# Atten4Vis/LW-DETR

Hardware: AMD Instinct MI355X
Metric: images/sec (higher is better)
Workload: dtype fp16; 1 GPU; LW-DETR-small inference forward + PostProcess, 640x640, batch 32/GPU, fp16, random-init weights (synthetic COCO-shaped input); global_batch=32, per_gpu_batch=32, parallelism=dp1, collective=none, launch_chains=2

## Files before the change

include/lwdetr_hip.h:

```cpp
#ifndef LWDETR_HIP_H
#define LWDETR_HIP_H
#include <stdint.h>
#ifdef __cplusplus
extern "C" {
#endif

#define LWDETR_OK 0
#define LWDETR_ERR_BAD_ARG (-1)
#define LWDETR_ERR_UNSUPPORTED (-2)
#define LWDETR_ERR_LAUNCH (-3)

int lwdetr_msda_forward(const void* value, const int64_t* shapes, const int64_t* level_start, const void* loc,
                        const void* attn, void* out, int B, int S, int M, int D, int L, int Q, int P, int dtype,
                        void* hip_stream);

int lwdetr_msda_backward(const void* value, const int64_t* shapes, const int64_t* level_start, const void* loc,
                         const void* attn, const void* grad_out, void* grad_value, void* grad_loc, void* grad_attn,
                         int B, int S, int M, int D, int L, int Q, int P, int dtype, void* hip_stream);

int lwdetr_msda_fused_forward(const void* value, const int64_t* shapes, const int64_t* level_start, const void* oa,
                              long ld_oa, int logit_col, const float* ref_boxes, const float* valid_ratios, void* out,
                              int B, int S, int M, int D, int L, int Q, int P, int dtype, void* hip_stream);

typedef struct {
// ... 41 lines not shown
    lwdetr_gemm_seg seg[3];
    void* splitk_ws;
    int splitk;
} lwdetr_gemm_desc;

int lwdetr_gemm(const lwdetr_gemm_desc* desc, int dtype, void* hip_stream);
int lwdetr_gemm_few(const lwdetr_gemm_desc* desc, int dtype, void* hip_stream);
int lwdetr_row_stats(const void* x, long ldx, long M, int C, float eps, float* stats, int dtype, void* hip_stream);
void lwdetr_gemm_tuning(int big_mode);
int lwdetr_has_experiments(void);
void lwdetr_gemm_pt_tuning(int pt_mode);
long lwdetr_gemm_pt_count(void);
int lwdetr_gemm_path_counts(long* out, int n);
const char* lwdetr_gemm_path_name(int i);

typedef struct {
    const void* Q;
    const void* K;
    const void* VT;
    void* out;
    long ldo;
    int B, heads, hd, Tp;
    int seqs_per_img;
    int seq_tok_stride;
    int keys_per_seq;
    int sub_stride, sub_len;
    int kind;
    int vt_slack;
} lwdetr_attn_desc;

int lwdetr_attention(const lwdetr_attn_desc* desc, int dtype, void* hip_stream);
void lwdetr_attention_tuning(int lds_mode);
void lwdetr_attention_tuning_cfg(int cfg);

int lwdetr_layernorm(const void* x, long ldx, const float* gamma, const float* beta, void* out, long ldo, long M,
                     int C, float eps, long rows_per_batch, long out_batch_rows, long out_row_offset, int dtype,
                     void* hip_stream);

int lwdetr_layernorm_chain(const void* x, long ldx, const float* gamma1, const float* beta1, float eps1, void* out1, long ldo1,
                           const float* gamma2, const float* beta2, float eps2, void* out2, long ldo2, long M, int C,
                           int dtype, void* hip_stream);

int lwdetr_ffn_splits(long M, int C, int hid, int dtype);
int lwdetr_ffn_partial(const void* x, long ldx, const void* w1, const float* b1, const void* w2_chunked, float* partial, long M,
                       int C, int hid, int dtype, void* hip_stream);
int lwdetr_ffn_finish(const void* x, long ldx, const float* partial, int splits, const float* b2, const float* gamma1,
                      const float* beta1, float eps1, void* out1, long ldo1, const float* gamma2, const float* beta2, float eps2,
                      void* out2, long ldo2, long M, int C, int dtype, void* hip_stream);

int lwdetr_mlp_fused(void* x, long ldx, const void* w1_folded, const float* b1_folded, const void* w2_chunked,
                     const float* b2, const float* gamma2, void* out2, long ld2, float* stats_out, long M, int C,
                     float eps, float eps_next, const void* att, long ldatt, const void* wp, const float* bp,
                     const float* gamma1, const void* wqkv_next, const float* bqkv_next, void* q_out, void* k_out,
                     void* vt_out, float qscale, int heads, int hd, int Tp, int dtype, void* hip_stream);

int lwdetr_vit_block_few(void* x, long ldx, const void* w1_frag, const float* b1_folded, const void* w2_chunked, const float* b2,
                         const float* gamma2, void* out2, long ld2, float* stats_out, long M, int C, float eps, float eps_next,
                         const void* att, long ldatt, const void* wp_frag, const float* bp, const float* gamma1,
                         const void* wqkv_frag_next, const float* bqkv_next, void* q_out, void* k_out, void* vt_out, float qscale,
                         int heads, int hd, int Tp, int dtype, void* hip_stream);

long lwdetr_vit_block_stream_bytes(int C, int has_qkv);
long lwdetr_vit_block_vec_floats(int C);
int lwdetr_vit_block(void* x, long ldx, const void* att, long ldatt, const void* wstream, const float* vec, void* out2,
                     long ld2, float* stats_out, long M, int C, float eps, float eps_next, int has_qkv, void* q_out,
                     void* k_out, void* vt_out, float qscale, int heads, int hd, int Tp, int dtype, void* hip_stream);
// ... 74 lines not shown
```

lw-detr_amd/csrc/attention.hip:

```cpp
#include "common.h"
#include <cstdlib>

namespace {

__device__ __forceinline__ float xor16_max(float v) {
    const auto r = __builtin_amdgcn_permlane16_swap(__float_as_uint(v), __float_as_uint(v), false, false);
    return fmaxf(__uint_as_float(r[0]), __uint_as_float(r[1]));
}
__device__ __forceinline__ float xor32_max(float v) {
    const auto r = __builtin_amdgcn_permlane32_swap(__float_as_uint(v), __float_as_uint(v), false, false);
    return fmaxf(__uint_as_float(r[0]), __uint_as_float(r[1]));
}
__device__ __forceinline__ float xor16_sum(float v) {
    const auto r = __builtin_amdgcn_permlane16_swap(__float_as_uint(v), __float_as_uint(v), false, false);
    return __uint_as_float(r[0]) + __uint_as_float(r[1]);
}
__device__ __forceinline__ float xor32_sum(float v) {
    const auto r = __builtin_amdgcn_permlane32_swap(__float_as_uint(v), __float_as_uint(v), false, false);
    return __uint_as_float(r[0]) + __uint_as_float(r[1]);
}

__device__ __forceinline__ float max3(float a, float b, float c) { return __builtin_fmaxf(__builtin_fmaxf(a, b), c); }

#ifndef LWDETR_ATTN_ABL
#define LWDETR_ATTN_ABL 0
#endif

template <typename T, int HD, int QT, bool SHORT = false>
__global__ __launch_bounds__(256) void attn_kernel(const lwdetr_attn_desc p) {
    typedef typename Vec<T>::v8 V8;
    typedef typename Vec<T>::v4 V4;
    constexpr int NC = HD >= 32 ? HD / 32 : 1;
    constexpr int DT = HD / 16;
    const int lane = threadIdx.x & 63, wave = threadIdx.x >> 6;
// ... 202 lines not shown
    }
}


template <typename T> struct Mma32;
template <> struct Mma32<f16> {
    static __device__ __forceinline__ f32x16 k16(f16x8 a, f16x8 b, f32x16 c) {
        return __builtin_amdgcn_mfma_f32_32x32x16_f16(a, b, c, 0, 0, 0);
    }
    static __device__ __forceinline__ float dot2(f16x8 p, int i, float c) {
        typedef _Float16 h2 __attribute__((ext_vector_type(2)));
        const h2 a = {p[2 * i], p[2 * i + 1]}, one = {(f16)1.f, (f16)1.f};
        return __builtin_amdgcn_fdot2(a, one, c, false);
    }
};
template <> struct Mma32<bf16> {
    static __device__ __forceinline__ f32x16 k16(bf16x8 a, bf16x8 b, f32x16 c) {
        return __builtin_amdgcn_mfma_f32_32x32x16_bf16(a, b, c, 0, 0, 0);
    }
    static __device__ __forceinline__ float dot2(bf16x8 p, int i, float c) {
        typedef __bf16 b2 __attribute__((ext_vector_type(2)));
        const b2 a = {p[2 * i], p[2 * i + 1]}, one = {(bf16)1.f, (bf16)1.f};
        return __builtin_amdgcn_fdot2_f32_bf16(a, one, c, false);
    }
};

__device__ __attribute__((aligned(16))) unsigned int g_attn_zero16[4];

__device__ __forceinline__ void attn_dma16(const void* src, unsigned lds_base) {
    asm volatile("s_mov_b32 m0, %0\n\ts_nop 0\n\tglobal_load_lds_dwordx4 %1, off" :: "s"(lds_base), "v"(src) : "memory");
}
template <int N> __device__ __forceinline__ void attn_wait_vmcnt() { asm volatile("s_waitcnt vmcnt(%0)" ::"n"(N) : "memory"); }

template <typename T, int HD, int QT, int NW, int U>
__global__ __launch_bounds__(NW * 64) void attn_lds_kernel(const lwdetr_attn_desc p) {
    typedef typename Vec<T>::v8 V8;
    constexpr int NC = HD / 16;
    constexpr int RT = HD > 32 ? HD / 32 : 1;
    constexpr int RB = HD * 2;
    constexpr int CPR = RB / 16, RPB = 256 / RB;
    constexpr int KB = 64;
    constexpr int KIMG = KB * RB, VIMG = RT * 32 * 128, STAGE = KIMG + VIMG;
    constexpr int NKP = KIMG / 1024, NVP = HD * 128 / 1024, NP = NKP + NVP;
    constexpr int SSTAGE = U * STAGE;
    constexpr int PPW = (U * NP + NW - 1) / NW;
    constexpr int NST = 3;
    constexpr int QW = 32 * QT, QWG = QW * NW;
    constexpr float RESCALE_THR = 8.f;
    __shared__ __attribute__((aligned(16))) char smem[NST * SSTAGE + 1024];

    const int lane = threadIdx.x & 63;
    const int wave = __builtin_amdgcn_readfirstlane(threadIdx.x >> 6);
    const int m = lane & 31, h = lane >> 5;
    const int nkeys = p.keys_per_seq;
    const int wgs_per_seq = (nkeys + QWG - 1) / QWG;
    int wid;
    {
        const int nwg = gridDim.x, bid = blockIdx.x, q = nwg >> 3, r = nwg & 7, xcd = bid & 7;
        wid = (xcd < r ? xcd * (q + 1) : r * (q + 1) + (xcd - r) * q) + (bid >> 3);
    }
    const int qblk = wid % wgs_per_seq;
    const int rest = wid / wgs_per_seq;
    const int head = rest % p.heads, seq = rest / p.heads;
    const int b = seq / p.seqs_per_img, w = seq - b * p.seqs_per_img;
    const long tok0 = (long)w * p.seq_tok_stride;
    const long bh = (long)b * p.heads + head;
    const T* __restrict__ Qb = (const T*)p.Q + (bh * p.Tp + tok0) * HD;
// ... 62 lines not shown
    const int km = (m & ~12) | ((m & 4) << 1) | ((m & 8) >> 1);
    int kofs[NC];
#pragma unroll
    for (int c = 0; c < NC; ++c) kofs[c] = km * RB + (((2 * c + h) ^ ((km / RPB) & (CPR - 1))) << 4);
    int vofs[2][2];
#pragma unroll
    for (int t = 0; t < 2; ++t)
#pragma unroll
        for (int s = 0; s < 2; ++s) vofs[t][s] = KIMG + m * 128 + (((4 * t + 2 * s + h) ^ ((m >> 1) & 7)) << 4);

    f32x16 o[QT][RT], negm[QT];
    float lsum[QT];
#pragma unroll
    for (int t = 0; t < QT; ++t) {
        lsum[t] = 0.f;
#pragma unroll
        for (int e = 0; e < 16; ++e) negm[t][e] = 0.f;
#pragma unroll
        for (int r = 0; r < RT; ++r)
#pragma unroll
            for (int e = 0; e < 16; ++e) o[t][r][e] = 0.f;
    }
    const bool holes = p.sub_len < p.sub_stride;
    int res0 = 0;

#pragma unroll
    for (int s = 0; s < NST - 1; ++s) issue(s, s);
#pragma unroll
    for (int t = 0; t < QT; ++t)
#pragma unroll
        for (int c = 0; c < NC; ++c) asm volatile("" :: "v"(qf[t][c]));

    int slot = 0;
    for (int ks = 0; ks < nstep; ++ks) {
        asm volatile("s_waitcnt lgkmcnt(0)" ::: "memory");
        attn_wait_vmcnt<(NST - 2) * PPW>();
        __builtin_amdgcn_s_barrier();
        {
            int ns = slot + NST - 1; ns = ns >= NST ? ns - NST : ns;
            issue(ks + NST - 1, ns);
        }
        const char* sS = smem + slot * SSTAGE;
        slot = slot + 1 == NST ? 0 : slot + 1;
#pragma unroll
        for (int u = 0; u < U; ++u) {
        const int kb = ks * U + u;
        if (kb >= nblk) break;
        const char* sK = sS + u * STAGE;
        if (active) {
#pragma unroll
            for (int t = 0; t < 2; ++t) {
                V8 kf[NC], vf[2][RT];
#pragma unroll
                for (int c = 0; c < NC; ++c) kf[c] = *(const V8*)(sK + t * 32 * RB + kofs[c]);
#pragma unroll
                for (int s = 0; s < 2; ++s)
#pragma unroll
                    for (int r = 0; r < RT; ++r) vf[s][r] = *(const V8*)(sK + r * 4096 + vofs[t][s]);
                f32x16 sc[QT];
#pragma unroll
                for (int qt = 0; qt < QT; ++qt) {
                    f32x16 a = negm[qt];
#pragma unroll
                    for (int c = 0; c < NC; ++c) a = Mma32<T>::k16(kf[c], qf[qt][c], a);
                    sc[qt] = a;
                }
// ... 28 lines not shown
                        float mx = xor32_max(lmax[qt]);
                        mx = first ? mx : fmaxf(mx, 0.f);
                        const float alpha = __builtin_amdgcn_exp2f(-mx);
#pragma unroll
                        for (int e = 0; e < 16; ++e) { negm[qt][e] -= mx; sc[qt][e] -= mx; }
                        lsum[qt] *= alpha;
#pragma unroll
                        for (int r = 0; r < RT; ++r)
#pragma unroll
                            for (int e = 0; e < 16; ++e) o[qt][r][e] *= alpha;
                    }
                }
#pragma unroll
                for (int qt = 0; qt < QT; ++qt) {
                    V8 pf[2];
#pragma unroll
                    for (int e = 0; e < 16; ++e) pf[e >> 3][e & 7] = from_f32<T>(__builtin_amdgcn_exp2f(sc[qt][e]));
                    if (HD > 16) {
#pragma unroll
                        for (int s = 0; s < 2; ++s)
#pragma unroll
                            for (int i = 0; i < 4; ++i) lsum[qt] = Mma32<T>::dot2(pf[s], i, lsum[qt]);
                    }
#pragma unroll
                    for (int s = 0; s < 2; ++s)
#pragma unroll
                        for (int r = 0; r < RT; ++r) o[qt][r] = Mma32<T>::k16(vf[s][r], pf[s], o[qt][r]);
                }
            }
        } else {
            res0 += 64; res0 %= p.sub_stride;
        }
        }
    }
    attn_wait_vmcnt<0>();
    if (!active) return;

    T* __restrict__ out = (T*)p.out;
#pragma unroll
    for (int qt = 0; qt < QT; ++qt) {
        float l;
        if (HD == 16) {
            const unsigned x = __float_as_uint(o[qt][0][8]);
            const auto rr = __builtin_amdgcn_permlane32_swap(x, x, false, false);
            l = __uint_as_float(rr[0]);
        } else {
            l = xor32_sum(lsum[qt]);
        }
        const float inv = 1.f / l;
        const int q = q0 + qt * 32 + m;
        T* orow = out + ((long)b * p.Tp + tok0 + q) * p.ldo + head * HD;
#pragma unroll
        for (int r = 0; r < RT; ++r)
#pragma unroll
            for (int j = 0; j < (HD == 16 ? 1 : 2); ++j) {
                typedef typename Vec<T>::v4 V4;
                V4 a4, b4;
#pragma unroll
                for (int e = 0; e < 4; ++e) {
                    a4[e] = from_f32<T>(o[qt][r][8 * j + e] * inv);
                    b4[e] = from_f32<T>(o[qt][r][8 * j + 4 + e] * inv);
                }
                typedef unsigned u2 __attribute__((ext_vector_type(2)));
                u2 au = __builtin_bit_cast(u2, a4), bu = __builtin_bit_cast(u2, b4);
#pragma unroll
                for (int d = 0; d < 2; ++d) {
                    const auto sw = __builtin_amdgcn_permlane32_swap(au[d], bu[d], false, false);
                    au[d] = sw[0]; bu[d] = sw[1];
                }
                typedef unsigned u4 __attribute__((ext_vector_type(4)));
                const u4 st = {au[0], au[1], bu[0], bu[1]};
                if (q < nkeys) *(u4*)(orow + r * 32 + j * 16 + h * 8) = st;
            }
    }
}

template <typename T, int HD, int QT, int NW, int U = 1>
int launch_lds(const lwdetr_attn_desc& p, hipStream_t st) {
    if constexpr (3 * U * (64 * HD * 2 + (HD > 32 ? HD / 32 : 1) * 32 * 128) + 1024 > 65536) return LWDETR_ERR_UNSUPPORTED;
    else {
    const int wgs_per_seq = (p.keys_per_seq + 32 * QT * NW - 1) / (32 * QT * NW);
    const long nwg = (long)wgs_per_seq * p.heads * p.B * p.seqs_per_img;
    const double nseq = (double)p.B * p.seqs_per_img;
    const double flops = 4.0 * nseq * p.heads * (double)p.keys_per_seq * p.keys_per_seq * HD;
    const double bytes = 4.0 * nseq * p.heads * p.keys_per_seq * HD * sizeof(T);
    ProfScope ps(p.kind == 0 ? KID_ATTN_WINDOW : (p.kind == 1 ? KID_ATTN_GLOBAL : KID_ATTN_DECODER), flops, bytes, st);
    hipLaunchKernelGGL((attn_lds_kernel<T, HD, QT, NW, U>), dim3((unsigned)nwg), dim3(NW * 64), 0, st, p);
    return lwdetr_check_launch();
    }
}

int g_attn_lds_cfg = 0;
}
extern "C" __attribute__((visibility("hidden"))) int lwdetr_attn_lds_hd16_impl(const lwdetr_attn_desc* p, int dtype, void* hip_stream, int cfg);
namespace {
template <typename T, int HD>
int launch_lds_cfg(const lwdetr_attn_desc& p, hipStream_t st) {
    int c = g_attn_lds_cfg ? g_attn_lds_cfg : (int)lwdetr_knob(KNOB_ATTN_LDS_CFG, 0);
#ifndef LWDETR_ATTN_HD16_TU
    if constexpr (HD == 16) return lwdetr_attn_lds_hd16_impl(&p, std::is_same<T, f16>::value ? DT_F16 : DT_BF16, (void*)st, c);
    else {
#else
    {
#endif
    if (!c) c = p.keys_per_seq <= 128 || HD == 16 ? 104 : (HD >= 64 && p.keys_per_seq >= 512 ? 208 : 108);
    switch (c) {
        case 102: return launch_lds<T, HD, 1, 2>(p, st);
        case 103: return launch_lds<T, HD, 1, 3>(p, st);
        case 104: return launch_lds<T, HD, 1, 4>(p, st);
        case 105: return launch_lds<T, HD, 1, 5>(p, st);
        case 106: return launch_lds<T, HD, 1, 6>(p, st);
        case 108: return launch_lds<T, HD, 1, 8>(p, st);
        case 110: return launch_lds<T, HD, 1, 10>(p, st);
        case 204: return launch_lds<T, HD, 2, 4>(p, st);
        case 205: return launch_lds<T, HD, 2, 5>(p, st);
        case 208: return launch_lds<T, HD, 2, 8>(p, st);
        case 1104: return launch_lds<T, HD, 1, 4, 2>(p, st);
        case 1105: return launch_lds<T, HD, 1, 5, 2>(p, st);
        case 1108: return launch_lds<T, HD, 1, 8, 2>(p, st);
        case 1110: return launch_lds<T, HD, 1, 10, 2>(p, st);
        case 3108: return launch_lds<T, HD, 1, 8, 4>(p, st);
        case 1208: return launch_lds<T, HD, 2, 8, 2>(p, st);
        default: return LWDETR_ERR_UNSUPPORTED;
    }
    }
}
template <typename T, int HD> struct LdsPath {
    static bool ok(const lwdetr_attn_desc&) { return false; }
    static int go(const lwdetr_attn_desc&, hipStream_t) { return LWDETR_ERR_UNSUPPORTED; }
};
template <int HD> struct LdsPath<f16, HD> {
    static bool ok(const lwdetr_attn_desc& p) { return true; }
    static int go(const lwdetr_attn_desc& p, hipStream_t st) { return launch_lds_cfg<f16, HD>(p, st); }
};
template <int HD> struct LdsPath<bf16, HD> {
    static bool ok(const lwdetr_attn_desc& p) { return true; }
    static int go(const lwdetr_attn_desc& p, hipStream_t st) { return launch_lds_cfg<bf16, HD>(p, st); }
};
// ... 365 lines not shown
    if constexpr (sizeof(T) == 2 && (HD == 16 || HD == 32)) {
        const int mode = (int)lwdetr_knob(KNOB_ATTN_WIN, 2);
        if (mode != 0 && (mode == 1 || HD == 32) && p.keys_per_seq <= 128 && p.sub_stride >= p.keys_per_seq && p.ldo % 8 == 0 &&
            ((size_t)p.out & 15) == 0 && (long)p.B * p.heads * p.seqs_per_img / 4 < 0x7fffffffL)
            return launch_win<T, HD>(p, st);
    }
    if (LdsPath<T, HD>::ok(p) && lds_path_applies(p)) return LdsPath<T, HD>::go(p, st);
    const long wgs4 = (long)((p.keys_per_seq + 255) / 256) * p.heads * p.B * p.seqs_per_img;
    const bool qt4 = lwdetr_knob_is_set(KNOB_ATTN_QT) ? lwdetr_knob(KNOB_ATTN_QT, 0) == 4 : (p.keys_per_seq >= 1024 && HD <= 32 && sizeof(T) == 2 && wgs4 >= 256);
    if (qt4) return launch_qt<T, HD, (HD <= 32 ? 4 : 2)>(p, st);
    return launch_qt<T, HD, 2>(p, st);
}

template <typename T>
int dispatch_hd(const lwdetr_attn_desc& p, hipStream_t st) {
    switch (p.hd) {
        case 16: return launch<T, 16>(p, st);
        case 32: return launch<T, 32>(p, st);
        case 64: return launch<T, 64>(p, st);
        default: return LWDETR_ERR_UNSUPPORTED;
    }
}

}

#ifdef LWDETR_ATTN_HD16_TU
extern "C" __attribute__((visibility("hidden"))) int lwdetr_attn_lds_hd16_impl(const lwdetr_attn_desc* p, int dtype, void* hip_stream, int cfg) {
    g_attn_lds_cfg = cfg;
    return dtype == DT_F16 ? launch_lds_cfg<f16, 16>(*p, (hipStream_t)hip_stream) : launch_lds_cfg<bf16, 16>(*p, (hipStream_t)hip_stream);
}
#else
extern "C" void lwdetr_attention_tuning(int lds_mode) { g_attn_lds_mode = lds_mode; }
extern "C" void lwdetr_attention_tuning_cfg(int cfg) { g_attn_lds_cfg = cfg; }

extern "C" int lwdetr_attention(const lwdetr_attn_desc* desc, int dtype, void* hip_stream) {
    if (!desc) return LWDETR_ERR_BAD_ARG;
    const lwdetr_attn_desc& p = *desc;
    if (!p.Q || !p.K || !p.VT || !p.out || p.B <= 0 || p.heads <= 0 || p.Tp <= 0 || p.Tp % 4 != 0) return LWDETR_ERR_BAD_ARG;
    if (p.seqs_per_img <= 0 || p.keys_per_seq < 8 || p.keys_per_seq % 4 != 0 || p.sub_stride <= 0 || p.sub_len <= 0 || p.sub_len > p.sub_stride)
        return LWDETR_ERR_BAD_ARG;
    if ((long)(p.seqs_per_img - 1) * p.seq_tok_stride + p.keys_per_seq > p.Tp) return LWDETR_ERR_BAD_ARG;
    if (p.seq_tok_stride % 4 != 0 || p.ldo % 4 != 0) return LWDETR_ERR_BAD_ARG;
    if ((long)p.B * p.seqs_per_img > 65535 || p.heads > 65535) return LWDETR_ERR_BAD_ARG;
    hipStream_t st = (hipStream_t)hip_stream;
    switch (dtype) {
        case DT_F32: return dispatch_hd<float>(p, st);
        case DT_F16: return dispatch_hd<f16>(p, st);
        case DT_BF16: return dispatch_hd<bf16>(p, st);
        default: return LWDETR_ERR_UNSUPPORTED;
    }
}
#endif
```

lw-detr_amd/csrc/vitblock.hip:

```cpp
#include "common.h"
#include <cstdlib>
#include <cstring>
#include <type_traits>

#ifndef LWDETR_VB_ABLATE
#define LWDETR_VB_ABLATE 0
#endif
#ifdef LWDETR_VB_TIMING
__device__ unsigned long long g_vb_timing[2][4][16];
#define VB_TS(i) do { if ((blockIdx.x == 0 || blockIdx.x == gridDim.x - 1) && lane == 0) { g_vb_timing[blockIdx.x != 0][wave][i] = __builtin_amdgcn_s_memrealtime(); \
    if ((i) == 0) g_vb_timing[blockIdx.x != 0][wave][12] = __builtin_amdgcn_s_memtime(); if ((i) == 11) g_vb_timing[blockIdx.x != 0][wave][15] = __builtin_amdgcn_s_memtime(); } } while (0)
extern "C" int lwdetr_debug_vb_timing(unsigned long long* out) {
    return hipMemcpyFromSymbol(out, HIP_SYMBOL(g_vb_timing), sizeof(g_vb_timing)) == hipSuccess ? 0 : 1;
}
#else
#define VB_TS(i) do {} while (0)
#endif

namespace {

template <typename T> struct Mma32;
template <> struct Mma32<f16> {
    static __device__ __forceinline__ f32x16 k16(f16x8 a, f16x8 b, f32x16 c) { return __builtin_amdgcn_mfma_f32_32x32x16_f16(a, b, c, 0, 0, 0); }
};
// ... 149 lines not shown
        if (ioff == NSLOT * PIECE_B) ioff = 0;
    };
    auto issued_is = [&](int n) { issued = n; isrc = wsrc + (size_t)n * PIECE_B; ioff = (unsigned)(n % NSLOT) * PIECE_B; };
#ifdef LWDETR_VB_TIMING
    unsigned long long tt_wait = 0, tt_bar = 0;
#endif
    auto boundary = [&](int a, int b, int extra) {
        __builtin_amdgcn_sched_barrier(0);
#ifdef LWDETR_VB_TIMING
        const unsigned long long ta = __builtin_amdgcn_s_memrealtime();
#endif
        vb_wait_le<(NSLOT - 4) * DPW>((issued - b) * DPW + extra);
#ifdef LWDETR_VB_TIMING
        const unsigned long long tb = __builtin_amdgcn_s_memrealtime();
#endif
        asm volatile("s_waitcnt lgkmcnt(0)" ::: "memory");
        __builtin_amdgcn_s_barrier();
#ifdef LWDETR_VB_TIMING
        tt_wait += tb - ta; tt_bar += __builtin_amdgcn_s_memrealtime() - tb;
#endif
        int lim = a + NSLOT; lim = lim < NP ? lim : NP;
#if LWDETR_VB_ABLATE & 4
        if (a >= H0) { issued = lim; return; }
#endif
        while (issued < lim) dma_next();
    };
    auto frag = [&](int piece, int f) -> V8 {
        return *(const V8*)(smem + ((unsigned)piece % NSLOT) * PIECE_B + f * 1024 + lane16);
    };
    auto frag_o = [&](unsigned off, int f) -> V8 { return *(const V8*)(smem + off + f * 1024 + lane16); };
    auto next_off = [](unsigned off) { off += PIECE_B; return off == NSLOT * PIECE_B ? 0u : off; };

    VB_TS(0);
    {
        const char* vsrc = (const char*)p.vec;
#pragma unroll
        for (int i = 0; i < VEC_DPW; ++i) {
            const unsigned kb = (unsigned)(wave * VEC_DPW + i) * 1024u;
            dma1k(vsrc, kb + lane16, lds0 + NSLOT * PIECE_B + kb);
        }
        while (issued < NSLOT) dma_next();
    }
    const T* att_w = (const T*)p.att + t0 * p.ldatt;
    T* x_w = (T*)p.x + t0 * p.ldx;
    const __amdgpu_buffer_rsrc_t r_att = __builtin_amdgcn_make_buffer_rsrc((void*)att_w, 0, (int)(nvalid * p.ldatt * 2), 0x00020000);
    const __amdgpu_buffer_rsrc_t r_x = __builtin_amdgcn_make_buffer_rsrc((void*)x_w, 0, (int)(nvalid * p.ldx * 2), 0x00020000);
    V8 xf[NH][KS];
#pragma unroll
    for (int th = 0; th < NH; ++th)
#pragma unroll
        for (int t = 0; t < KS; ++t)
            xf[th][t] = __builtin_bit_cast(V8, __builtin_amdgcn_raw_buffer_load_b128(
                r_att, (unsigned)(((32 * th + j) * p.ldatt + 16 * t + 8 * h) * 2), 0, 0));

    f32x16 acc2[NTI][NH];
    {
        u32x4 xv[NH][NTI][2];
#pragma unroll
        for (int th = 0; th < NH; ++th)
#pragma unroll
            for (int n = 0; n < NTI; ++n)
#pragma unroll
                for (int jb = 0; jb < 2; ++jb)
                    xv[th][n][jb] = __builtin_amdgcn_raw_buffer_load_b128(
                        r_x, (unsigned)(((32 * th + j) * p.ldx + 32 * n + 16 * jb + 8 * h) * 2), 0, 0);
        boundary(0, 2, NH * KS + NH * NTI * 2);
        VB_TS(1);
#pragma unroll
        for (int n = 0; n < NTI; ++n) {
            f32x16 na[NH];
#pragma unroll
            for (int jb = 0; jb < 2; ++jb)
#pragma unroll
                for (int th = 0; th < NH; ++th) {
                    const u32x4 own = vb_rows8(xv[th][n][jb][0], xv[th][n][jb][1], xv[th][n][jb][2], xv[th][n][jb][3]);
#pragma unroll
                    for (int bb = 0; bb < 2; ++bb) {
                        const int b = 2 * jb + bb, c0 = 32 * n + 8 * b + 4 * h;
                        const f32x4 bbv = *(const f32x4*)(bps + c0), rg = *(const f32x4*)(rg1s + c0);
#pragma unroll
                        for (int d = 0; d < 2; ++d) {
                            const unsigned ow_ = own[2 * bb + d];
                            const typename Pk<T>::v2 v2 = __builtin_bit_cast(typename Pk<T>::v2, ow_);
                            na[th][4 * b + 2 * d] = fmaf(to_f32<T>(v2[0]), rg[2 * d], bbv[2 * d]);
                            na[th][4 * b + 2 * d + 1] = fmaf(to_f32<T>(v2[1]), rg[2 * d + 1], bbv[2 * d + 1]);
                        }
                    }
                }
#pragma unroll
            for (int th = 0; th < NH; ++th) {
                asm volatile("" : "+a"(na[th]));
                acc2[n][th] = na[th];
            }
            __builtin_amdgcn_sched_barrier(0);
        }
    }
    VB_TS(2);
#pragma unroll
    for (int s = 0; s < NTI / 2; ++s) {
        if (s > 0) boundary(2 * s, 2 * s + 2, 2 * s + 1 < NSLOT ? NH * KS + NH * NTI * 2 : 0);
        {
            V8 fr[RD];
#pragma unroll
            for (int i = 0; i < RD; ++i) fr[i] = frag(2 * s + i / KS, i % KS);
#pragma unroll
            for (int fi = 0; fi < 2 * KS; ++fi) {
                const int n = 2 * s + fi / KS, t = fi % KS;
                const V8 a = fr[fi % RD];
#pragma unroll
                for (int th = 0; th < NH; ++th) acc2[n][th] = Mma32<T>::k16(a, xf[th][t], acc2[n][th]);
                if (fi + RD < 2 * KS) fr[fi % RD] = frag(2 * s + (fi + RD) / KS, (fi + RD) % KS);
                __builtin_amdgcn_sched_barrier(0);
            }
        }
    }
    VB_TS(3);
    auto unpack2 = [](unsigned w, float& a, float& b) {
        const typename Pk<T>::v2 v = __builtin_bit_cast(typename Pk<T>::v2, w);
        a = to_f32<T>(v[0]); b = to_f32<T>(v[1]);
    };
#pragma unroll
    for (int th = 0; th < NH; ++th) {
        unsigned xp[NTI][8];
        float s = 0.f;
#pragma unroll
        for (int n = 0; n < NTI; ++n) {
#pragma unroll
            for (int b = 0; b < 4; ++b) {
                const f32x4 gg = *(const f32x4*)(g1s + 32 * n + 8 * b + 4 * h);
#pragma unroll
                for (int d = 0; d < 2; ++d) {
                    const unsigned w = pack2<T>(gg[2 * d] * acc2[n][th][4 * b + 2 * d], gg[2 * d + 1] * acc2[n][th][4 * b + 2 * d + 1]);
                    xp[n][2 * b + d] = w;
// ... 165 lines not shown
    iter(I0{}, No{}, Yes{}, 0u, (unsigned)((H0 + 1) % NSLOT) * PIECE_B, 0);
    VB_TS(6);
#ifdef LWDETR_VB_TIMING
    tt_wait = 0; tt_bar = 0;
#endif
    unsigned co = (unsigned)((H0 + 2) % NSLOT) * PIECE_B;
#pragma unroll 1
    for (int k = 1; k < NCH - 1; k += 2) {
        boundary(H0 + 2 * k, H0 + 2 * k + 2, 0);
        { const unsigned o1 = next_off(co); iter(I1{}, Yes{}, Yes{}, co, o1, k); co = next_off(o1); }
        boundary(H0 + 2 * k + 2, H0 + 2 * k + 4, 0);
        { const unsigned o1 = next_off(co); iter(I0{}, Yes{}, Yes{}, co, o1, k + 1); co = next_off(o1); }
    }
    VB_TS(7);
#ifdef LWDETR_VB_TIMING
    if ((blockIdx.x == 0 || blockIdx.x == gridDim.x - 1) && lane == 0) { g_vb_timing[blockIdx.x != 0][wave][13] = tt_wait; g_vb_timing[blockIdx.x != 0][wave][14] = tt_bar; }
#endif
    { constexpr int il = H0 + 2 * NCH - 4 + NSLOT; issued_is(il < NP ? il : NP); }
    boundary(H0 + 2 * NCH - 2, H0 + 2 * NCH - 1, 0);
    iter(I1{}, Yes{}, No{}, (unsigned)((H0 + 2 * NCH - 2) % NSLOT) * PIECE_B, 0u, NCH - 1);
    VB_TS(8);
    {
        boundary(H0 + 2 * NCH - 1, H0 + 2 * NCH, 0);
#pragma unroll
        for (int fi = 0; fi < 2 * NTI; ++fi) {
            const V8 a = frag(H0 + 2 * NCH - 1, fi);
            const int kap = fi / NTI, n = fi % NTI;
#pragma unroll
            for (int th = 0; th < NH; ++th) acc2[n][th] = Mma32<T>::k16(a, __builtin_bit_cast(V8, hf[1][th][kap]), acc2[n][th]);
        }
    }

    VB_TS(9);
    const __amdgpu_buffer_rsrc_t r_o2 = __builtin_amdgcn_make_buffer_rsrc(
        p.out2 ? (void*)((T*)p.out2 + t0 * p.ld2) : (void*)x_w, 0, p.out2 ? (int)(nvalid * p.ld2 * 2) : 0, 0x00020000);
    const bool has_o2 = p.out2 != nullptr;
#pragma unroll
    for (int th = 0; th < NH; ++th) {
        float s = 0.f;
#pragma unroll
        for (int n = 0; n < NTI; ++n) {
#pragma unroll
            for (int jb = 0; jb < 2; ++jb) {
                unsigned pw[4];
#pragma unroll
                for (int bb = 0; bb < 2; ++bb) {
                    const int b = 2 * jb + bb;
                    const f32x4 gg = *(const f32x4*)(g2s + 32 * n + 8 * b + 4 * h);
#pragma unroll
                    for (int d = 0; d < 2; ++d) {
                        const unsigned w = pack2<T>(gg[2 * d] * acc2[n][th][4 * b + 2 * d], gg[2 * d + 1] * acc2[n][th][4 * b + 2 * d + 1]);
                        pw[2 * bb + d] = w;
                        const typename Pk<T>::v2 v2 = __builtin_bit_cast(typename Pk<T>::v2, w);
                        const float v0 = to_f32<T>(v2[0]), v1 = to_f32<T>(v2[1]);
                        acc2[n][th][4 * b + 2 * d] = v0; acc2[n][th][4 * b + 2 * d + 1] = v1;
                        s += v0 + v1;
                    }
                }
                const u32x4 ow = vb_rows8(pw[0], pw[1], pw[2], pw[3]);
                const int c0 = 32 * n + 16 * jb + 8 * h;
                __builtin_amdgcn_raw_buffer_store_b128(ow, r_x, (unsigned)(((32 * th + j) * p.ldx + c0) * 2), 0, 0);
                if (has_o2) __builtin_amdgcn_raw_buffer_store_b128(ow, r_o2, (unsigned)(((32 * th + j) * p.ld2 + c0) * 2), 0, 0);
            }
            __builtin_amdgcn_sched_barrier(0);
        }
        if (p.stats_out || QKV) {
            s += __shfl_xor(s, 32);
            const float mean = s * (1.f / C);
            float v = 0.f;
#pragma unroll
            for (int n = 0; n < NTI; ++n)
#pragma unroll
                for (int e = 0; e < 16; ++e) { const float dl = acc2[n][th][e] - mean; v += dl * dl; }
            v += __shfl_xor(v, 32);
            const float rstd = 1.f / sqrtf(v * (1.f / C) + p.eps_next), nmr = -mean * rstd;
            if (p.stats_out && h == 0 && 32 * th + j < nvalid) {
                float* so = p.stats_out + 2 * (t0 + 32 * th + j);
                so[0] = mean; so[1] = rstd;
            }
            if (QKV) {
#pragma unroll
                for (int n = 0; n < NTI; ++n)
#pragma unroll
                    for (int be = 0; be < 2; ++be)
                        {
                            u32x4 w;
#pragma unroll
                            for (int d = 0; d < 4; ++d) {
                                const int r = (2 * be + (d >> 1)) * 4 + (d & 1) * 2;
                                w[d] = pack2<T>(fmaf(acc2[n][th][r], rstd, nmr), fmaf(acc2[n][th][r + 1], rstd, nmr));
                            }
                            xf[th][2 * n + be] = __builtin_bit_cast(V8, w);
                        }
            }
        }
    }

    VB_TS(10);
    if (QKV) {
        const __amdgpu_buffer_rsrc_t r_q = __builtin_amdgcn_make_buffer_rsrc(p.q, 0, (int)p.qkv_bytes, 0x00020000);
        const __amdgpu_buffer_rsrc_t r_k = __builtin_amdgcn_make_buffer_rsrc(p.k, 0, (int)p.qkv_bytes, 0x00020000);
        const __amdgpu_buffer_rsrc_t r_v = __builtin_amdgcn_make_buffer_rsrc(p.vt, 0, (int)p.qkv_bytes, 0x00020000);
        const int hd = 1 << p.hd_log2;
        auto qk_col = [&](int f) -> unsigned { return (unsigned)((((long)(f >> p.hd_log2) * p.Tp) << p.hd_log2) + (f & (hd - 1))); };
        unsigned vo_qk[NH];
#pragma unroll
        for (int th = 0; th < NH; ++th) {
            const unsigned tok = (unsigned)t0 + 32 * th + j;
            const unsigned img = tok / (unsigned)p.Tp, wi = tok - img * (unsigned)p.Tp;
            vo_qk[th] = 32 * th + j < nvalid ? ((unsigned)(((long)img * p.heads * p.Tp + wi) << p.hd_log2) + qk_col(8 * h)) * 2u : 0x80000000u;
        }
        constexpr int XST = NH * NTI * 2, SPS = 2 * NH * 2, LAG = (NSLOT - 2) / 2;
        const int est = XST * (has_o2 ? 2 : 1);
        unsigned vo_v[NH][2];
#pragma unroll
        for (int th = 0; th < NH; ++th)
#pragma unroll
            for (int jb = 0; jb < 2; ++jb) {
                const int tl = 32 * th + 16 * jb + 8 * h;
                const unsigned tk = (unsigned)t0 + tl;
                const unsigned im = tk / (unsigned)p.Tp, wv = tk - im * (unsigned)p.Tp;
                vo_v[th][jb] = tl < nvalid ? ((unsigned)((long)im * p.heads * hd * p.Tp + wv) + (unsigned)j * (unsigned)p.Tp) * 2u : 0x80000000u;
            }
#pragma unroll
        for (int th = 0; th < NH; ++th) asm volatile("" : "+v"(vo_qk[th]), "+v"(vo_v[th][0]), "+v"(vo_v[th][1]));
        constexpr int NS = NP_QKV / 2, NGR = 4 * NH, SLOTS = 2 * KS, GAP = SLOTS / NGR, NLAY = 6;
        constexpr int RDQ = 4;
        static_assert(NTI % 2 == 0 && SLOTS % NGR == 0 && GAP >= 3, "both pieces of a step belong to one of q / k / v");
        f32x16 qacc[2][2][NH];
        float gv[8];
        f32x4 gb0, gb1;
        float gbv = 0.f;
        auto layer = [&](auto sh_tag, auto g_tag, auto l_tag) {
            constexpr int sh = decltype(sh_tag)::value, BUF = sh & 1, g = decltype(g_tag)::value, L = decltype(l_tag)::value;
            constexpr int pp = g / (2 * NH), jb = (g / NH) % 2, th = g % NH;
            constexpr int pi = 2 * sh + pp, sg = pi / NTI, nl0 = (pi - sg * NTI) * 32;
            if constexpr (L <= 1) asm volatile("" : "+a"(qacc[BUF][pp][th]));
            else asm volatile("" : "+v"(gv[0]), "+v"(gv[1]), "+v"(gv[2]), "+v"(gv[3]), "+v"(gv[4]), "+v"(gv[5]), "+v"(gv[6]), "+v"(gv[7]));
            if constexpr (L == 0) {
#pragma unroll
                for (int e = 0; e < 4; ++e) gv[e] = qacc[BUF][pp][th][8 * jb + e];
                if constexpr (sg < 2) {
                    gb0 = *(const f32x4*)(bqs + sg * C + nl0 + 16 * jb + 4 * h);
                    gb1 = *(const f32x4*)(bqs + sg * C + nl0 + 16 * jb + 8 + 4 * h);
                } else {
                    unsigned ln;
                    asm volatile("v_mbcnt_lo_u32_b32 %0, -1, 0\n\tv_mbcnt_hi_u32_b32 %0, -1, %0" : "=v"(ln));
                    gbv = bqs[2 * C + nl0 + (int)(ln & 31u)];
                }
            } else if constexpr (L == 1) {
#pragma unroll
                for (int e = 0; e < 4; ++e) gv[4 + e] = qacc[BUF][pp][th][8 * jb + 4 + e];
            } else if constexpr (L == 2) {
#pragma unroll
                for (int e = 0; e < 4; ++e) gv[e] += sg < 2 ? gb0[e] : gbv;
            } else if constexpr (L == 3) {
#pragma unroll
                for (int e = 0; e < 4; ++e) gv[4 + e] += sg < 2 ? gb1[e] : gbv;
            } else if constexpr (L == 4) {
                if constexpr (sg == 0) {
#pragma unroll
                    for (int e = 0; e < 8; ++e) gv[e] *= p.qscale;
                }
            } else {
                const u32x4 ow = vb_rows8(pack2<T>(gv[0], gv[1]), pack2<T>(gv[2], gv[3]), pack2<T>(gv[4], gv[5]), pack2<T>(gv[6], gv[7]));
                if constexpr (sg < 2) {
                    const unsigned so = __builtin_amdgcn_readfirstlane(qk_col(nl0 + 16 * jb) * 2u);
                    if constexpr (sg == 0) __builtin_amdgcn_raw_buffer_store_b128(ow, r_q, vo_qk[th], so, 0);
                    else __builtin_amdgcn_raw_buffer_store_b128(ow, r_k, vo_qk[th], so, 0);
                } else {
                    const unsigned so = __builtin_amdgcn_readfirstlane((unsigned)nl0 * (unsigned)p.Tp * 2u);
                    __builtin_amdgcn_raw_buffer_store_b128(ow, r_v, vo_v[th][jb], so, 0);
                }
            }
            if constexpr (L < NLAY - 1)
                asm volatile("" : "+v"(gv[0]), "+v"(gv[1]), "+v"(gv[2]), "+v"(gv[3]), "+v"(gv[4]), "+v"(gv[5]), "+v"(gv[6]), "+v"(gv[7]));
        };
// ... 745 lines not shown
```

Before: 14150 images/sec.

## Add software-pipelined key loop to LDS attention kernel for hd16 sequences

Adds a PIPE variant of the LDS flash-attention kernel that software-pipelines the key loop. It computes the next 32-key QK^T MFMA while doing softmax exp and PV MFMAs for the current tile, and prefetches the next K fragments across the ring-buffer barrier. It becomes the default for hd16 when the config is 104, there are no holes and keys are a multiple of 64. The aim is to hide MFMA and LDS latency behind exp work. In exchange it uses more registers and restricts the path to QT=1, U=1. It also records the last launched config for introspection.

Result: faster. 14320 images/sec (median of 6 runs) (+1.2%).

```diff
diff --git a/include/lwdetr_hip.h b/include/lwdetr_hip.h
--- a/include/lwdetr_hip.h
+++ b/include/lwdetr_hip.h
@@ -97,6 +97,7 @@
 int lwdetr_attention(const lwdetr_attn_desc* desc, int dtype, void* hip_stream);
 void lwdetr_attention_tuning(int lds_mode);
 void lwdetr_attention_tuning_cfg(int cfg);
+int lwdetr_attention_last_lds_cfg(void);
 
 int lwdetr_layernorm(const void* x, long ldx, const float* gamma, const float* beta, void* out, long ldo, long M,
                      int C, float eps, long rows_per_batch, long out_batch_rows, long out_row_offset, int dtype,
diff --git a/lw-detr_amd/csrc/attention.hip b/lw-detr_amd/csrc/attention.hip
--- a/lw-detr_amd/csrc/attention.hip
+++ b/lw-detr_amd/csrc/attention.hip
@@ -1,5 +1,6 @@
 #include "common.h"
 #include <cstdlib>
+#include <type_traits>
 
 namespace {
 
@@ -268,7 +269,7 @@
 }
 template <int N> __device__ __forceinline__ void attn_wait_vmcnt() { asm volatile("s_waitcnt vmcnt(%0)" ::"n"(N) : "memory"); }
 
-template <typename T, int HD, int QT, int NW, int U>
+template <typename T, int HD, int QT, int NW, int U, int PIPE>
 __global__ __launch_bounds__(NW * 64) void attn_lds_kernel(const lwdetr_attn_desc p) {
     typedef typename Vec<T>::v8 V8;
     constexpr int NC = HD / 16;
@@ -397,6 +398,96 @@
         for (int c = 0; c < NC; ++c) asm volatile("" :: "v"(qf[t][c]));
 
     int slot = 0;
+    if constexpr (PIPE != 0) {
+    static_assert(QT == 1 && U == 1 && RT == 1, "the pipelined key loop: 32 queries per wave, 64 keys per ring step, hd <= 32");
+    const char* sS = smem;
+    auto enter = [&](int ks) {
+        asm volatile("s_waitcnt lgkmcnt(0)" ::: "memory");
+        attn_wait_vmcnt<(NST - 2) * PPW>();
+        __builtin_amdgcn_s_barrier();
+        int ns = slot + NST - 1; ns = ns >= NST ? ns - NST : ns;
+        issue(ks + NST - 1, ns);
+        sS = smem + slot * SSTAGE;
+        slot = slot + 1 == NST ? 0 : slot + 1;
+    };
+    if (!active) {
+        for (int ks = 0; ks <= nstep; ++ks) enter(ks);
+    } else {
+        f32x16 sc;
+        V8 vf[2][2];
+        enter(0);
+        {
+            V8 kf[NC];
+#pragma unroll
+            for (int c = 0; c < NC; ++c) kf[c] = *(const V8*)(sS + kofs[c]);
+            sc = negm[0];
+#pragma unroll
+            for (int c = 0; c < NC; ++c) sc = Mma32<T>::k16(kf[c], qf[0][c], sc);
+        }
+        auto tile = [&](auto t_, auto first_, int ks) {
+            constexpr int t = decltype(t_)::value;
+            constexpr bool first = decltype(first_)::value;
+            V8 kn[NC], pf[2];
+            if (t == 0) {
+#pragma unroll
+                for (int tt = 0; tt < 2; ++tt)
+#pragma unroll
+                    for (int s = 0; s < 2; ++s) vf[tt][s] = *(const V8*)(sS + vofs[tt][s]);
+            }
+            float lm = max3(sc[0], sc[1], sc[2]);
+#pragma unroll
+            for (int e = 3; e < 15; e += 2) lm = max3(lm, sc[e], sc[e + 1]);
+            lm = __builtin_fmaxf(lm, sc[15]);
+            asm volatile("" :: "v"(lm));
+            __builtin_amdgcn_sched_barrier(0);
+            const char* sN = sS + 32 * RB;
+            if (t == 1) {
+                enter(ks + 1);
+                sN = sS;
+            }
+#pragma unroll
+            for (int c = 0; c < NC; ++c) kn[c] = *(const V8*)(sN + kofs[c]);
+            __builtin_amdgcn_sched_barrier(0);
+            if (first || __any(lm > RESCALE_THR)) {
+                float mx = xor32_max(lm);
+                mx = first ? mx : fmaxf(mx, 0.f);
+                const float alpha = __builtin_amdgcn_exp2f(-mx);
+#pragma unroll
+                for (int e = 0; e < 16; ++e) { negm[0][e] -= mx; sc[e] -= mx; }
+                lsum[0] *= alpha;
+#pragma unroll
+                for (int e = 0; e < 16; ++e) o[0][0][e] *= alpha;
+            }
+#pragma unroll
+            for (int e = 0; e < 8; ++e) pf[0][e] = from_f32<T>(__builtin_amdgcn_exp2f(sc[e]));
+            __builtin_amdgcn_sched_barrier(0);
+            f32x16 sn = negm[0];
+#pragma unroll
+            for (int c = 0; c < NC; ++c) sn = Mma32<T>::k16(kn[c], qf[0][c], sn);
+            if (HD > 16) {
+#pragma unroll
+                for (int i = 0; i < 4; ++i) lsum[0] = Mma32<T>::dot2(pf[0], i, lsum[0]);
+            }
+            o[0][0] = Mma32<T>::k16(vf[t][0], pf[0], o[0][0]);
+            __builtin_amdgcn_sched_barrier(0);
+#pragma unroll
+            for (int e = 0; e < 8; ++e) pf[1][e] = from_f32<T>(__builtin_amdgcn_exp2f(sc[8 + e]));
+            if (HD > 16) {
+#pragma unroll
+                for (int i = 0; i < 4; ++i) lsum[0] = Mma32<T>::dot2(pf[1], i, lsum[0]);
+            }
+            o[0][0] = Mma32<T>::k16(vf[t][1], pf[1], o[0][0]);
+            sc = sn;
+        };
+        typedef std::integral_constant<int, 0> T0; typedef std::integral_constant<int, 1> T1;
+        tile(T0(), std::true_type(), 0);
+        tile(T1(), std::false_type(), 0);
+        for (int ks = 1; ks < nstep; ++ks) {
+            tile(T0(), std::false_type(), ks);
+            tile(T1(), std::false_type(), ks);
+        }
+    }
+    } else {
     for (int ks = 0; ks < nstep; ++ks) {
         asm volatile("s_waitcnt lgkmcnt(0)" ::: "memory");
         attn_wait_vmcnt<(NST - 2) * PPW>();
@@ -491,6 +582,7 @@
             res0 += 64; res0 %= p.sub_stride;
         }
         }
+    }
     }
     attn_wait_vmcnt<0>();
     if (!active) return;
@@ -534,8 +626,15 @@
     }
 }
 
-template <typename T, int HD, int QT, int NW, int U = 1>
+}
+extern "C" __attribute__((visibility("hidden"))) int lwdetr_attn_lds_last_cfg;
+#ifndef LWDETR_ATTN_HD16_TU
+int lwdetr_attn_lds_last_cfg = 0;
+#endif
+namespace {
+template <typename T, int HD, int QT, int NW, int U = 1, int PIPE = 0>
 int launch_lds(const lwdetr_attn_desc& p, hipStream_t st) {
+    if (PIPE != 0 && (p.sub_len != p.sub_stride || p.keys_per_seq % 64 != 0)) return LWDETR_ERR_UNSUPPORTED;
     if constexpr (3 * U * (64 * HD * 2 + (HD > 32 ? HD / 32 : 1) * 32 * 128) + 1024 > 65536) return LWDETR_ERR_UNSUPPORTED;
     else {
     const int wgs_per_seq = (p.keys_per_seq + 32 * QT * NW - 1) / (32 * QT * NW);
@@ -544,7 +643,8 @@
     const double flops = 4.0 * nseq * p.heads * (double)p.keys_per_seq * p.keys_per_seq * HD;
     const double bytes = 4.0 * nseq * p.heads * p.keys_per_seq * HD * sizeof(T);
     ProfScope ps(p.kind == 0 ? KID_ATTN_WINDOW : (p.kind == 1 ? KID_ATTN_GLOBAL : KID_ATTN_DECODER), flops, bytes, st);
-    hipLaunchKernelGGL((attn_lds_kernel<T, HD, QT, NW, U>), dim3((unsigned)nwg), dim3(NW * 64), 0, st, p);
+    hipLaunchKernelGGL((attn_lds_kernel<T, HD, QT, NW, U, PIPE>), dim3((unsigned)nwg), dim3(NW * 64), 0, st, p);
+    lwdetr_attn_lds_last_cfg = 10000 * PIPE + 1000 * (U - 1) + 100 * QT + NW;
     return lwdetr_check_launch();
     }
 }
@@ -556,6 +656,7 @@
 template <typename T, int HD>
 int launch_lds_cfg(const lwdetr_attn_desc& p, hipStream_t st) {
     int c = g_attn_lds_cfg ? g_attn_lds_cfg : (int)lwdetr_knob(KNOB_ATTN_LDS_CFG, 0);
+    const int c0 = c;
 #ifndef LWDETR_ATTN_HD16_TU
     if constexpr (HD == 16) return lwdetr_attn_lds_hd16_impl(&p, std::is_same<T, f16>::value ? DT_F16 : DT_BF16, (void*)st, c);
     else {
@@ -563,6 +664,11 @@
     {
 #endif
     if (!c) c = p.keys_per_seq <= 128 || HD == 16 ? 104 : (HD >= 64 && p.keys_per_seq >= 512 ? 208 : 108);
+    if (!c0 && c == 104 && HD == 16 && p.sub_len == p.sub_stride && p.keys_per_seq % 64 == 0) c = 10104;
+    if constexpr (HD <= 32) {
+        if (c == 10104) return launch_lds<T, HD, 1, 4, 1, 1>(p, st);
+        if (c == 10108) return launch_lds<T, HD, 1, 8, 1, 1>(p, st);
+    }
     switch (c) {
         case 102: return launch_lds<T, HD, 1, 2>(p, st);
         case 103: return launch_lds<T, HD, 1, 3>(p, st);
@@ -994,6 +1100,7 @@
 #else
 extern "C" void lwdetr_attention_tuning(int lds_mode) { g_attn_lds_mode = lds_mode; }
 extern "C" void lwdetr_attention_tuning_cfg(int cfg) { g_attn_lds_cfg = cfg; }
+extern "C" int lwdetr_attention_last_lds_cfg(void) { return lwdetr_attn_lds_last_cfg; }
 
 extern "C" int lwdetr_attention(const lwdetr_attn_desc* desc, int dtype, void* hip_stream) {
     if (!desc) return LWDETR_ERR_BAD_ARG;
```

## Issue activation loads before LDS DMA prologue and recompute lane ids in epilogue

Applied to the files above, without the earlier changes.

Moves the residual (x) and attention fragment global loads ahead of the LDS DMA prologue, issues only two DMA pieces up front, then drains all vmcnt with an explicit s_waitcnt. The intent is to get the register-destined loads in flight earlier and stop boundary() from carrying vmcnt counts for them. The epilogue now recomputes lane row/half indices with mbcnt and replaces __shfl_xor with a direct ds_bpermute, which lowers register pressure across the long main loop. In exchange, the full drain stalls until every load lands, and fewer DMA pieces are in flight during the first stage.

After: 14340 images/sec before, 14360 images/sec after (median of 4 runs). Within noise of the previous version (+0.1%).

```diff
diff --git a/lw-detr_amd/csrc/vitblock.hip b/lw-detr_amd/csrc/vitblock.hip
--- a/lw-detr_amd/csrc/vitblock.hip
+++ b/lw-detr_amd/csrc/vitblock.hip
@@ -205,39 +205,40 @@
     auto next_off = [](unsigned off) { off += PIECE_B; return off == NSLOT * PIECE_B ? 0u : off; };
 
     VB_TS(0);
-    {
-        const char* vsrc = (const char*)p.vec;
-#pragma unroll
-        for (int i = 0; i < VEC_DPW; ++i) {
-            const unsigned kb = (unsigned)(wave * VEC_DPW + i) * 1024u;
-            dma1k(vsrc, kb + lane16, lds0 + NSLOT * PIECE_B + kb);
-        }
-        while (issued < NSLOT) dma_next();
-    }
     const T* att_w = (const T*)p.att + t0 * p.ldatt;
     T* x_w = (T*)p.x + t0 * p.ldx;
     const __amdgpu_buffer_rsrc_t r_att = __builtin_amdgcn_make_buffer_rsrc((void*)att_w, 0, (int)(nvalid * p.ldatt * 2), 0x00020000);
     const __amdgpu_buffer_rsrc_t r_x = __builtin_amdgcn_make_buffer_rsrc((void*)x_w, 0, (int)(nvalid * p.ldx * 2), 0x00020000);
     V8 xf[NH][KS];
+    u32x4 xv[NH][NTI][2];
+#pragma unroll
+    for (int th = 0; th < NH; ++th)
+#pragma unroll
+        for (int n = 0; n < NTI; ++n)
+#pragma unroll
+            for (int jb = 0; jb < 2; ++jb)
+                xv[th][n][jb] = __builtin_amdgcn_raw_buffer_load_b128(
+                    r_x, (unsigned)(((32 * th + j) * p.ldx + 32 * n + 16 * jb + 8 * h) * 2), 0, 0);
 #pragma unroll
     for (int th = 0; th < NH; ++th)
 #pragma unroll
         for (int t = 0; t < KS; ++t)
             xf[th][t] = __builtin_bit_cast(V8, __builtin_amdgcn_raw_buffer_load_b128(
                 r_att, (unsigned)(((32 * th + j) * p.ldatt + 16 * t + 8 * h) * 2), 0, 0));
+    {
+        const char* vsrc = (const char*)p.vec;
+#pragma unroll
+        for (int i = 0; i < VEC_DPW; ++i) {
+            const unsigned kb = (unsigned)(wave * VEC_DPW + i) * 1024u;
+            dma1k(vsrc, kb + lane16, lds0 + NSLOT * PIECE_B + kb);
+        }
+        while (issued < 2) dma_next();
+    }
+    __builtin_amdgcn_s_waitcnt(0x0F70);
 
     f32x16 acc2[NTI][NH];
     {
-        u32x4 xv[NH][NTI][2];
-#pragma unroll
-        for (int th = 0; th < NH; ++th)
-#pragma unroll
-            for (int n = 0; n < NTI; ++n)
-#pragma unroll
-                for (int jb = 0; jb < 2; ++jb)
-                    xv[th][n][jb] = __builtin_amdgcn_raw_buffer_load_b128(
-                        r_x, (unsigned)(((32 * th + j) * p.ldx + 32 * n + 16 * jb + 8 * h) * 2), 0, 0);
-        boundary(0, 2, NH * KS + NH * NTI * 2);
+        boundary(0, 2, 0);
         VB_TS(1);
 #pragma unroll
         for (int n = 0; n < NTI; ++n) {
@@ -271,7 +272,7 @@
     VB_TS(2);
 #pragma unroll
     for (int s = 0; s < NTI / 2; ++s) {
-        if (s > 0) boundary(2 * s, 2 * s + 2, 2 * s + 1 < NSLOT ? NH * KS + NH * NTI * 2 : 0);
+        if (s > 0) boundary(2 * s, 2 * s + 2, 0);
         {
             V8 fr[RD];
 #pragma unroll
@@ -503,6 +504,12 @@
     }
 
     VB_TS(9);
+    unsigned lne;
+    asm volatile("v_mbcnt_lo_u32_b32 %0, -1, 0\n\tv_mbcnt_hi_u32_b32 %0, -1, %0" : "=v"(lne));
+    const int je = (int)(lne & 31u), he = (int)(lne >> 5);
+    auto other_half = [&](float v) -> float {
+        return __builtin_bit_cast(float, __builtin_amdgcn_ds_bpermute((int)((lne ^ 32u) << 2), __builtin_bit_cast(int, v)));
+    };
     const __amdgpu_buffer_rsrc_t r_o2 = __builtin_amdgcn_make_buffer_rsrc(
         p.out2 ? (void*)((T*)p.out2 + t0 * p.ld2) : (void*)x_w, 0, p.out2 ? (int)(nvalid * p.ld2 * 2) : 0, 0x00020000);
     const bool has_o2 = p.out2 != nullptr;
@@ -517,7 +524,7 @@
 #pragma unroll
                 for (int bb = 0; bb < 2; ++bb) {
                     const int b = 2 * jb + bb;
-                    const f32x4 gg = *(const f32x4*)(g2s + 32 * n + 8 * b + 4 * h);
+                    const f32x4 gg = *(const f32x4*)(g2s + 32 * n + 8 * b + 4 * he);
 #pragma unroll
                     for (int d = 0; d < 2; ++d) {
                         const unsigned w = pack2<T>(gg[2 * d] * acc2[n][th][4 * b + 2 * d], gg[2 * d + 1] * acc2[n][th][4 * b + 2 * d + 1]);
@@ -529,24 +536,24 @@
                     }
                 }
                 const u32x4 ow = vb_rows8(pw[0], pw[1], pw[2], pw[3]);
-                const int c0 = 32 * n + 16 * jb + 8 * h;
-                __builtin_amdgcn_raw_buffer_store_b128(ow, r_x, (unsigned)(((32 * th + j) * p.ldx + c0) * 2), 0, 0);
-                if (has_o2) __builtin_amdgcn_raw_buffer_store_b128(ow, r_o2, (unsigned)(((32 * th + j) * p.ld2 + c0) * 2), 0, 0);
+                const int c0 = 32 * n + 16 * jb + 8 * he;
+                __builtin_amdgcn_raw_buffer_store_b128(ow, r_x, (unsigned)(((32 * th + je) * p.ldx + c0) * 2), 0, 0);
+                if (has_o2) __builtin_amdgcn_raw_buffer_store_b128(ow, r_o2, (unsigned)(((32 * th + je) * p.ld2 + c0) * 2), 0, 0);
             }
             __builtin_amdgcn_sched_barrier(0);
         }
         if (p.stats_out || QKV) {
-            s += __shfl_xor(s, 32);
+            s += other_half(s);
             const float mean = s * (1.f / C);
             float v = 0.f;
 #pragma unroll
             for (int n = 0; n < NTI; ++n)
 #pragma unroll
                 for (int e = 0; e < 16; ++e) { const float dl = acc2[n][th][e] - mean; v += dl * dl; }
-            v += __shfl_xor(v, 32);
+            v += other_half(v);
             const float rstd = 1.f / sqrtf(v * (1.f / C) + p.eps_next), nmr = -mean * rstd;
-            if (p.stats_out && h == 0 && 32 * th + j < nvalid) {
-                float* so = p.stats_out + 2 * (t0 + 32 * th + j);
+            if (p.stats_out && he == 0 && 32 * th + je < nvalid) {
+                float* so = p.stats_out + 2 * (t0 + 32 * th + je);
                 so[0] = mean; so[1] = rstd;
             }
             if (QKV) {
@@ -577,9 +584,9 @@
         unsigned vo_qk[NH];
 #pragma unroll
         for (int th = 0; th < NH; ++th) {
-            const unsigned tok = (unsigned)t0 + 32 * th + j;
+            const unsigned tok = (unsigned)t0 + 32 * th + je;
             const unsigned img = tok / (unsigned)p.Tp, wi = tok - img * (unsigned)p.Tp;
-            vo_qk[th] = 32 * th + j < nvalid ? ((unsigned)(((long)img * p.heads * p.Tp + wi) << p.hd_log2) + qk_col(8 * h)) * 2u : 0x80000000u;
+            vo_qk[th] = 32 * th + je < nvalid ? ((unsigned)(((long)img * p.heads * p.Tp + wi) << p.hd_log2) + qk_col(8 * he)) * 2u : 0x80000000u;
         }
         constexpr int XST = NH * NTI * 2, SPS = 2 * NH * 2, LAG = (NSLOT - 2) / 2;
         const int est = XST * (has_o2 ? 2 : 1);
@@ -588,10 +595,10 @@
         for (int th = 0; th < NH; ++th)
 #pragma unroll
             for (int jb = 0; jb < 2; ++jb) {
-                const int tl = 32 * th + 16 * jb + 8 * h;
+                const int tl = 32 * th + 16 * jb + 8 * he;
                 const unsigned tk = (unsigned)t0 + tl;
                 const unsigned im = tk / (unsigned)p.Tp, wv = tk - im * (unsigned)p.Tp;
-                vo_v[th][jb] = tl < nvalid ? ((unsigned)((long)im * p.heads * hd * p.Tp + wv) + (unsigned)j * (unsigned)p.Tp) * 2u : 0x80000000u;
+                vo_v[th][jb] = tl < nvalid ? ((unsigned)((long)im * p.heads * hd * p.Tp + wv) + (unsigned)je * (unsigned)p.Tp) * 2u : 0x80000000u;
             }
 #pragma unroll
         for (int th = 0; th < NH; ++th) asm volatile("" : "+v"(vo_qk[th]), "+v"(vo_v[th][0]), "+v"(vo_v[th][1]));
@@ -612,8 +619,8 @@
 #pragma unroll
                 for (int e = 0; e < 4; ++e) gv[e] = qacc[BUF][pp][th][8 * jb + e];
                 if constexpr (sg < 2) {
-                    gb0 = *(const f32x4*)(bqs + sg * C + nl0 + 16 * jb + 4 * h);
-                    gb1 = *(const f32x4*)(bqs + sg * C + nl0 + 16 * jb + 8 + 4 * h);
+                    gb0 = *(const f32x4*)(bqs + sg * C + nl0 + 16 * jb + 4 * he);
+                    gb1 = *(const f32x4*)(bqs + sg * C + nl0 + 16 * jb + 8 + 4 * he);
                 } else {
                     unsigned ln;
                     asm volatile("v_mbcnt_lo_u32_b32 %0, -1, 0\n\tv_mbcnt_hi_u32_b32 %0, -1, %0" : "=v"(ln));
```
